# esrice/trio_binning

Measured on AMD Instinct MI355X. Metric: Gbases/sec classified (k=21, 2x300M k-mer tables), higher is better.
Workload: dtype u64

## Files before the change

### trio_binning_amd/csrc/tbk_host.cpp

```cpp
#include <hip/hip_runtime.h>

#include <fcntl.h>
#include <sys/mman.h>
#include <sys/stat.h>
#include <unistd.h>

#include <algorithm>
#include <chrono>
#include <cmath>
#include <cerrno>
#include <cstdarg>
#include <cstdio>
#include <cstdlib>
#include <cstring>
#include <cctype>
#include <pthread.h>
#include <sched.h>
#include <atomic>
#include <memory>
#include <mutex>
#include <string>
#include <thread>
#include <vector>

// ... 189 lines not shown
    buf[got] = 0;
    int n = 0;
    const char *p = buf;
    while (*p) {
        while (*p == ',' || *p == ' ' || *p == '\n') p++;
        if (!isdigit((unsigned char)*p)) break;
        char *end = nullptr;
        long lo = strtol(p, &end, 10), hi = lo;
        p = end;
        if (*p == '-') { hi = strtol(p + 1, &end, 10); p = end; }
        for (long c = lo; c <= hi && c < CPU_SETSIZE; c++) { if (cpus && n < cap) cpus[n] = (int)c; n++; }
    }
    return n;
}

extern "C" int tbk_numa_bind_thread_(int node) {
    const char *off = getenv("TBK_NUMA");
    if (off && *off == '0') return 0;
    std::vector<int> cpus(CPU_SETSIZE);
    const int n = tbk_numa_node_cpus_(node, cpus.data(), (int)cpus.size());
    if (n <= 0) return 0;
    cpu_set_t cur, want;
    if (pthread_getaffinity_np(pthread_self(), sizeof cur, &cur) != 0) return 0;
    CPU_ZERO(&want);
    for (int i = 0; i < std::min(n, (int)cpus.size()); i++) if (CPU_ISSET(cpus[(size_t)i], &cur)) CPU_SET(cpus[(size_t)i], &want);
    const int k = CPU_COUNT(&want);
    if (k == 0 || k == CPU_COUNT(&cur)) return k == 0 ? 0 : k;
    if (pthread_setaffinity_np(pthread_self(), sizeof want, &want) != 0) return 0;
    return k;
}

extern "C" int tbk_device_numa_node(int device, int *node) {
    if (!node) return fail(TBK_ERR_INVALID, "node is NULL");
    *node = -1;
    char bdf[64] = {0};
    int n_visible = 0;
    if (hipGetDeviceCount(&n_visible) != hipSuccess || n_visible <= 0) { (void)hipGetLastError(); return fail(TBK_ERR_NO_DEVICE, "no HIP device visible"); }
    if (device < 0 || device >= n_visible) return fail(TBK_ERR_INVALID, "device %d out of range (0..%d)", device, n_visible - 1);
    if (hipDeviceGetPCIBusId(bdf, (int)sizeof bdf, device) != hipSuccess) { (void)hipGetLastError(); return TBK_OK; }
    *node = tbk_numa_node_of_pci_(bdf);
    return TBK_OK;
}

extern "C" int tbk_numa_bind_to_device(int device, int *node_out, int *cpus_out) {
    int node = -1;
    const int rc = tbk_device_numa_node(device, &node);
    if (node_out) *node_out = node;
    if (cpus_out) *cpus_out = 0;
    if (rc) return rc;
    const int k = tbk_numa_bind_thread_(node);
    if (cpus_out) *cpus_out = k;
    return TBK_OK;
}

static void table_born();
static void table_gone();
struct tbk_table {
    tbk_table() { table_born(); }
    ~tbk_table() { table_gone(); }
    tbk_table(const tbk_table &) = delete;
    tbk_table &operator=(const tbk_table &) = delete;
    int device = 0;
    int k = 0;
    uint64_t num_lines = 0;
    int origin = 0;
    uint64_t *d_keys = nullptr;
    uint64_t *d_slots = nullptr;
    uint32_t n_buckets = 0;
    uint64_t distinct = 0;
    bool hashed = false;
    TbkTableView view() const { return TbkTableView{d_slots, n_buckets, 8, 0, TbkMz{0, 0, 0, 0}, 0}; }
};

struct ListRef {
    const uint64_t *d_keys;
    uint64_t num_lines;
    ListRef(const tbk_table *t) : d_keys(t->d_keys), num_lines(t->num_lines) {}
    ListRef(const uint64_t *keys, uint64_t n) : d_keys(keys), num_lines(n) {}
    const ListRef *operator->() const { return this; }
};

static constexpr int RING = 3;
static constexpr int TIMING_POOL = 4096;

struct Slot {
    uint8_t *d_bases = nullptr; size_t cap_bases = 0;
    uint64_t *d_offsets = nullptr; size_t cap_reads = 0;
    int32_t *d_counts = nullptr;
    uint8_t *h_bases = nullptr; size_t hcap_bases = 0;
    uint64_t *h_offsets = nullptr; int32_t *h_counts = nullptr; size_t hcap_reads = 0;
    uint32_t *d_codes = nullptr; uint16_t *d_bad = nullptr; size_t cap_chunks = 0;
    bool bad_clean = false;
    uint32_t *d_exc_chunk = nullptr; uint16_t *d_exc_mask = nullptr; size_t cap_exc = 0;
    uint32_t *h_codes = nullptr; size_t hcap_chunks = 0;
    uint32_t *h_exc_chunk = nullptr; uint16_t *h_exc_mask = nullptr; size_t hcap_exc = 0;
    hipEvent_t copied = nullptr, probed = nullptr, done = nullptr, copied2 = nullptr;
    hipEvent_t sliced[8] = {nullptr, nullptr, nullptr, nullptr, nullptr, nullptr, nullptr, nullptr};
    bool busy = false;
    uint64_t ticket = 0, n_reads = 0;
    int32_t *user_counts = nullptr;
    bool counts_staged = false;
};

struct DeviceStreams {
    int device = 0;
    hipStream_t compute = nullptr, copy = nullptr, out = nullptr;
    hipStream_t copy2 = nullptr;
    std::mutex enqueue;
    std::atomic<int> in_flight{0};
    ~DeviceStreams() {
        if (hipSetDevice(device) != hipSuccess) return;
        if (compute) (void)hipStreamDestroy(compute);
        if (copy) (void)hipStreamDestroy(copy);
        if (copy2) (void)hipStreamDestroy(copy2);
        if (out) (void)hipStreamDestroy(out);
    }
};

struct tbk_classifier {
    int device = 0;
    int k = 0;
    tbk_options opt = resolve_options(nullptr);
    std::shared_ptr<DeviceStreams> streams;
    uint64_t *d_pair = nullptr;
    std::shared_ptr<uint64_t> pair_owner;
    void *pair_base = nullptr;
    void own_pair() {
        const int dev = device;
        void *base = pair_base ? pair_base : (void *)d_pair;
        pair_owner = std::shared_ptr<uint64_t>(d_pair, [dev, base](uint64_t *) { if (base && hipSetDevice(dev) == hipSuccess) (void)hipFree(base); });
        pair_base = nullptr;
    }
    hipError_t alloc_pair(size_t bytes) {
        const size_t align = (size_t)opt.table_align;
        pair_base = nullptr; d_pair = nullptr;
        hipError_t e = hipMalloc(&pair_base, bytes + align);
        if (e != hipSuccess) { pair_base = nullptr; return e; }
        uintptr_t p = (uintptr_t)pair_base;
        if (align > 1) p = (p + align - 1) / align * align;
        d_pair = (uint64_t *)p;
        return hipSuccess;
    }
    void free_pair() {
        if (pair_base) (void)hipFree(pair_base);
        else if (d_pair) (void)hipFree(d_pair);
        pair_base = nullptr; d_pair = nullptr;
    }
    uint32_t n_buckets = 0;
    uint64_t distinct_a = 0, distinct_b = 0;
    uint64_t shared = 0;
    TbkMz mz{0, 0, 0};
    int replica_copies = 0;
    int layout_builds = 0;
    uint64_t past_half = 0;
    uint64_t behind_front = 0;
    uint64_t entries_a = 0, entries_b = 0;
    uint32_t guests = 0;
    uint64_t verified_lines = 0;
    double verify_s = 0;
    uint32_t over_mask = 0;
    uint64_t table_bytes() const { return (uint64_t)n_buckets * 2 * TBK_BUCKET_BYTES + ((guests & TBK_FLAG_SHORT) ? ((uint64_t)over_mask + 1) * 8 : 0); }
    TbkPairView pair() const { return TbkPairView{d_pair, n_buckets, mz, guests, over_mask}; }
    hipStream_t compute = nullptr, copy = nullptr, out = nullptr;
    Slot ring[RING];
    uint64_t next_ticket = 1;
    int max_blocks = 0;
// ... 1462 lines not shown
    if (e == hipSuccess) e = hipEventRecord(e0, c->compute);
    if (e == hipSuccess) e = tbk_launch_gather_pairs(c->d_pair, bytes, inflight, waves_per_simd, n_lines, 9, sink, &done, c->compute);
    if (e == hipSuccess) e = hipEventRecord(e1, c->compute);
    if (e == hipSuccess) e = hipEventSynchronize(e1);
    if (e == hipSuccess) e = hipEventElapsedTime(&ms, e0, e1);
    if (e0) (void)hipEventDestroy(e0);
    if (e1) (void)hipEventDestroy(e1);
    (void)hipFree(sink);
    if (e != hipSuccess) return fail(e == hipErrorInvalidValue ? TBK_ERR_INVALID : TBK_ERR_HIP, "tbk_classifier_calibrate_pairs: %s", hipGetErrorString(e));
    *lines_per_sec = ms > 0 ? (double)done / (ms * 1e-3) : 0;
    return TBK_OK;
}

extern "C" int tbk_classifier_table_id(const tbk_classifier *c, uint64_t *table_id, int *is_replica) {
    if (!c) return fail(TBK_ERR_INVALID, "classifier is NULL");
    if (table_id) *table_id = (uint64_t)(uintptr_t)c->d_pair;
    if (is_replica) *is_replica = c->replica_copies;
    return TBK_OK;
}

extern "C" int tbk_classifier_shared_keys(const tbk_classifier *c, uint64_t *n_shared) {
    if (!c || !n_shared) return fail(TBK_ERR_INVALID, "NULL argument");
    *n_shared = c->shared;
    return TBK_OK;
}

extern "C" void tbk_classifier_destroy(tbk_classifier *c) {
    if (!c) return;
    if (hipSetDevice(c->device) == hipSuccess) {
        if (c->compute) (void)hipStreamSynchronize(c->compute);
        if (c->copy) (void)hipStreamSynchronize(c->copy);
        if (c->out) (void)hipStreamSynchronize(c->out);
        for (Slot &s : c->ring) {
            if (s.d_bases) (void)hipFree(s.d_bases);
            if (s.d_offsets) (void)hipFree(s.d_offsets);
            if (s.d_counts) (void)hipFree(s.d_counts);
            if (s.h_bases) (void)hipHostFree(s.h_bases);
            if (s.h_offsets) (void)hipHostFree(s.h_offsets);
            if (s.h_counts) (void)hipHostFree(s.h_counts);
            if (s.d_codes) (void)hipFree(s.d_codes);
            if (s.d_bad) (void)hipFree(s.d_bad);
            if (s.d_exc_chunk) (void)hipFree(s.d_exc_chunk);
            if (s.d_exc_mask) (void)hipFree(s.d_exc_mask);
            if (s.h_codes) (void)hipHostFree(s.h_codes);
            if (s.h_exc_chunk) (void)hipHostFree(s.h_exc_chunk);
            if (s.h_exc_mask) (void)hipHostFree(s.h_exc_mask);
            if (s.copied) (void)hipEventDestroy(s.copied);
            if (s.probed) (void)hipEventDestroy(s.probed);
            if (s.done) (void)hipEventDestroy(s.done);
            if (s.copied2) (void)hipEventDestroy(s.copied2);
            for (hipEvent_t e : s.sliced) if (e) (void)hipEventDestroy(e);
        }
        for (hipEvent_t e : c->ev) (void)hipEventDestroy(e);
        c->pair_owner.reset();
        if (c->d_pass_read) (void)hipFree(c->d_pass_read);
        c->small_free();
        for (const Slot &s : c->ring) if (s.busy && c->streams) c->streams->in_flight--;
        c->streams.reset();
    }
    delete c;
}

static void par_memcpy(void *dst, const void *src, size_t n) {
    const size_t piece = (size_t)16 << 20;
    const int nt = (int)std::min<size_t>((size_t)tbk_host_threads(), n / piece);
    if (nt <= 1) { memcpy(dst, src, n); return; }
    std::vector<std::thread> pool;
    for (int t = 0; t < nt; t++) {
        const size_t lo = n * (size_t)t / nt, hi = n * (size_t)(t + 1) / nt;
        pool.emplace_back([=]() { memcpy((char *)dst + lo, (const char *)src + lo, hi - lo); });
    }
    for (std::thread &th : pool) th.join();
}

static bool is_pinned(const void *p) {
    hipPointerAttribute_t at;
    hipError_t e = hipPointerGetAttributes(&at, p);
    if (e != hipSuccess) { (void)hipGetLastError(); return false; }
    return at.type == hipMemoryTypeHost;
}

struct ProbeSlice { uint64_t pass_lo, pass_hi; hipEvent_t arrived; };

static int launch_probe_timed(tbk_classifier *c, const uint8_t *d_bases, const uint64_t *d_offsets,
                              uint64_t n_reads, uint64_t total, int32_t *d_counts, const uint32_t *d_codes = nullptr,
                              const uint16_t *d_bad16 = nullptr, const ProbeSlice *slices = nullptr, int n_slices = 0) {
    if (n_reads >= 0xFFFFFFF0ull) return fail(TBK_ERR_INVALID, "more than 2^32 reads in one batch");
    if (total == 0) {
        HIP_TRY(hipMemsetAsync(d_counts, 0, n_reads * 2 * sizeof(int32_t), c->compute));
        return TBK_OK;
    }
    const uint64_t passes = tbk_probe_passes(total);
    if (passes > c->cap_passes) {
        HIP_TRY(hipStreamSynchronize(c->compute));
        if (c->d_pass_read) HIP_TRY(hipFree(c->d_pass_read));
        c->d_pass_read = nullptr; c->cap_passes = 0;
        const uint64_t cap = (passes + passes / 4 + 1024 + 1) & ~1ull;
        HIP_TRY(hipMalloc((void **)&c->d_pass_read, (4 * cap + 16) * sizeof(uint32_t)));
        c->cap_passes = cap;
    }
    const ProbeSlice whole = {0, passes, nullptr};
    if (n_slices <= 0) { slices = &whole; n_slices = 1; }
    hipEvent_t *ev = nullptr;
    if (c->timing) {
        const size_t need = 2 + 3 * (size_t)n_slices;
        if (c->ev_used + need > c->ev.size() && c->ev.size() >= (size_t)TIMING_POOL) {
            HIP_TRY(hipStreamSynchronize(c->compute));
            int rc = c->fold_timing();
            if (rc) return rc;
        }
        while (c->ev_used + need > c->ev.size()) {
            hipEvent_t a;
            HIP_TRY(hipEventCreate(&a));
            c->ev.push_back(a);
        }
        ev = c->ev.data() + c->ev_used;
        c->ev_used += need;
        c->ev_slices.push_back((uint32_t)n_slices);
        c->timed_launches++;
        HIP_TRY(hipEventRecord(ev[0], c->compute));
    }
    HIP_TRY(tbk_launch_probe_index(d_offsets, n_reads, total, d_counts, c->d_pass_read, c->cap_passes, c->opt.two_read_kernel != 0 && tbk_probe_has_two_read_kernel(c->mz), c->compute));
    if (ev) HIP_TRY(hipEventRecord(ev[1], c->compute));
    for (int j = 0; j < n_slices; j++) {
        if (slices[j].arrived) HIP_TRY(hipStreamWaitEvent(c->compute, slices[j].arrived, 0));
        if (ev) HIP_TRY(hipEventRecord(ev[2 + 3 * j], c->compute));
        HIP_TRY(tbk_launch_probe_range(d_bases, d_codes, d_bad16, d_offsets, n_reads, total, c->pair(), c->k, d_counts, c->d_pass_read, c->cap_passes,
                                       slices[j].pass_lo, slices[j].pass_hi, c->max_blocks, c->opt.two_read_kernel != 0, ev ? ev[3 + 3 * j] : nullptr, c->compute, 0));
        if (ev) HIP_TRY(hipEventRecord(ev[4 + 3 * j], c->compute));
    }
    c->last_passes = passes;
    return TBK_OK;
}

int tbk_classifier::fold_timing() {
    size_t at = 0;
    for (uint32_t n_slices : ev_slices) {
        float ms = 0;
        HIP_TRY(hipEventElapsedTime(&ms, ev[at], ev[at + 1]));
        timed_ms += ms;
        for (uint32_t j = 0; j < n_slices; j++) {
            float whole = 0, single = 0;
            HIP_TRY(hipEventElapsedTime(&whole, ev[at + 2 + 3 * j], ev[at + 4 + 3 * j]));
            HIP_TRY(hipEventElapsedTime(&single, ev[at + 3 + 3 * j], ev[at + 4 + 3 * j]));
            timed_ms += whole;
            timed_single_ms += single;
        }
        at += 2 + 3 * (size_t)n_slices;
    }
    ev_used = 0;
    ev_slices.clear();
    return TBK_OK;
}

extern "C" int tbk_stream_depth(const tbk_classifier *) { return RING; }

extern "C" int tbk_check_offsets_(const uint64_t *offsets, uint64_t n_reads) {
    if (!offsets) return fail(TBK_ERR_INVALID, "offsets is NULL");
    if (offsets[0] != 0) return fail(TBK_ERR_INVALID, "offsets[0] must be 0");
    for (uint64_t i = 0; i < n_reads; i++)
        if (offsets[i + 1] < offsets[i]) return fail(TBK_ERR_INVALID, "offsets not non-decreasing at read %llu", (unsigned long long)i);
    return TBK_OK;
}

static int slot_reserve_device(Slot &s, uint64_t total, uint64_t n_reads) {
    const size_t need_b = ((size_t)total + 15) & ~(size_t)15;
    if (need_b > s.cap_bases) {
        if (s.d_bases) HIP_TRY(hipFree(s.d_bases));
        s.d_bases = nullptr; s.cap_bases = 0;
        const size_t cap = std::max(need_b + need_b / 8, (size_t)1 << 20);
        HIP_TRY(hipMalloc((void **)&s.d_bases, cap));
        s.cap_bases = cap;
    }
    if (n_reads > s.cap_reads) {
        if (s.d_offsets) HIP_TRY(hipFree(s.d_offsets));
        if (s.d_counts) HIP_TRY(hipFree(s.d_counts));
        s.d_offsets = nullptr; s.d_counts = nullptr; s.cap_reads = 0;
        const size_t cap = std::max((size_t)n_reads + (size_t)n_reads / 8, (size_t)1024);
        HIP_TRY(hipMalloc((void **)&s.d_offsets, (cap + 1) * sizeof(uint64_t)));
        HIP_TRY(hipMalloc((void **)&s.d_counts, cap * 2 * sizeof(int32_t)));
        s.cap_reads = cap;
    }
    return TBK_OK;
}

static int slot_reserve(Slot &s, uint64_t stage_bases, uint64_t n_reads, bool stage_small, bool stage_out) {
    const size_t need_b = ((size_t)stage_bases + 15) & ~(size_t)15;
    if (need_b > s.hcap_bases) {
        if (s.h_bases) HIP_TRY(hipHostFree(s.h_bases));
        s.h_bases = nullptr; s.hcap_bases = 0;
        const size_t cap = std::max(need_b + need_b / 8, (size_t)1 << 20);
        HIP_TRY(hipHostMalloc((void **)&s.h_bases, cap, hipHostMallocPortable));
        s.hcap_bases = cap;
    }
    if ((stage_small || stage_out) && n_reads > s.hcap_reads) {
        if (s.h_offsets) HIP_TRY(hipHostFree(s.h_offsets));
        if (s.h_counts) HIP_TRY(hipHostFree(s.h_counts));
        s.h_offsets = nullptr; s.h_counts = nullptr; s.hcap_reads = 0;
        const size_t cap = std::max((size_t)n_reads + (size_t)n_reads / 8, (size_t)1024);
        HIP_TRY(hipHostMalloc((void **)&s.h_offsets, (cap + 1) * sizeof(uint64_t), hipHostMallocPortable));
        HIP_TRY(hipHostMalloc((void **)&s.h_counts, cap * 2 * sizeof(int32_t), hipHostMallocPortable));
        s.hcap_reads = cap;
    }
    return TBK_OK;
}

static int slot_reserve_packed(Slot &s, uint64_t n_chunks, uint64_t n_exc) {
    if (n_chunks > s.cap_chunks) {
        if (s.d_codes) HIP_TRY(hipFree(s.d_codes));
        if (s.d_bad) HIP_TRY(hipFree(s.d_bad));
        s.d_codes = nullptr; s.d_bad = nullptr; s.cap_chunks = 0;
        const size_t cap = std::max((size_t)n_chunks + (size_t)n_chunks / 8, (size_t)1 << 16);
        HIP_TRY(hipMalloc((void **)&s.d_codes, cap * sizeof(uint32_t)));
        HIP_TRY(hipMalloc((void **)&s.d_bad, (cap + 2) * sizeof(uint16_t)));
        s.cap_chunks = cap;
        s.bad_clean = false;
    }
    if (n_exc > s.cap_exc) {
        if (s.d_exc_chunk) HIP_TRY(hipFree(s.d_exc_chunk));
        if (s.d_exc_mask) HIP_TRY(hipFree(s.d_exc_mask));
        s.d_exc_chunk = nullptr; s.d_exc_mask = nullptr; s.cap_exc = 0;
        const size_t cap = std::max((size_t)n_exc + (size_t)n_exc / 4, (size_t)4096);
        HIP_TRY(hipMalloc((void **)&s.d_exc_chunk, cap * sizeof(uint32_t)));
        HIP_TRY(hipMalloc((void **)&s.d_exc_mask, cap * sizeof(uint16_t)));
        s.cap_exc = cap;
    }
    return TBK_OK;
}

static int slot_reserve_packed_host(Slot &s, uint64_t n_chunks, uint64_t n_exc) {
    if (n_chunks > s.hcap_chunks) {
// ... 8 lines not shown
        if (s.h_exc_mask) HIP_TRY(hipHostFree(s.h_exc_mask));
        s.h_exc_chunk = nullptr; s.h_exc_mask = nullptr; s.hcap_exc = 0;
        const size_t cap = std::max((size_t)n_exc + (size_t)n_exc / 4, (size_t)4096);
        HIP_TRY(hipHostMalloc((void **)&s.h_exc_chunk, cap * sizeof(uint32_t), hipHostMallocPortable));
        HIP_TRY(hipHostMalloc((void **)&s.h_exc_mask, cap * sizeof(uint16_t), hipHostMallocPortable));
        s.hcap_exc = cap;
    }
    return TBK_OK;
}

static int submit_host(tbk_classifier *c, const uint8_t *bases, const uint32_t *codes, const uint32_t *exc_chunk, const uint16_t *exc_mask,
                       uint64_t n_exc, const uint64_t *offsets, uint64_t n_reads, int32_t *counts, uint64_t *ticket) {
    if (!c || !offsets || !ticket || (n_reads && !counts)) return fail(TBK_ERR_INVALID, "NULL argument");
    int rc = tbk_check_offsets_(offsets, n_reads);
    if (rc) return rc;
    const uint64_t total = offsets[n_reads];
    if (total && !bases && !codes) return fail(TBK_ERR_INVALID, "bases is NULL");
    if (codes && n_exc && (!exc_chunk || !exc_mask)) return fail(TBK_ERR_INVALID, "exception arrays are NULL");
    rc = use_device(c->device);
    if (rc) return rc;
    const uint64_t tk = c->next_ticket;
    Slot &s = c->ring[tk % RING];
    if (s.busy) return fail(TBK_ERR_STATE, "all %d stream slots are in flight; call tbk_stream_wait(%llu) first", RING,
                            (unsigned long long)s.ticket);
    const uint64_t n_chunks = tbk_packed_chunks(total);
    bool packed = codes != nullptr;
    if (!packed && total && c->packed_h2d) {
        rc = slot_reserve_packed_host(s, n_chunks, 0);
        if (rc) return rc;
        rc = tbk_pack_bases_vec(bases, total, s.h_codes, c->exc_chunk, c->exc_mask, c->pack_threads);
        if (rc) return fail(rc, "%s", g_err.c_str());
        n_exc = c->exc_chunk.size();
        rc = slot_reserve_packed_host(s, n_chunks, n_exc);
        if (rc) return rc;
        if (n_exc) {
            memcpy(s.h_exc_chunk, c->exc_chunk.data(), n_exc * sizeof(uint32_t));
            memcpy(s.h_exc_mask, c->exc_mask.data(), n_exc * sizeof(uint16_t));
        }
        codes = s.h_codes; exc_chunk = s.h_exc_chunk; exc_mask = s.h_exc_mask;
        packed = true;
    } else if (packed && total) {
        const bool codes_pinned = is_pinned(codes), exc_pinned = n_exc == 0 || (is_pinned(exc_chunk) && is_pinned(exc_mask));
        rc = slot_reserve_packed_host(s, codes_pinned ? 0 : n_chunks, exc_pinned ? 0 : n_exc);
        if (rc) return rc;
        if (!codes_pinned) { par_memcpy(s.h_codes, codes, n_chunks * sizeof(uint32_t)); codes = s.h_codes; }
        if (!exc_pinned) {
            memcpy(s.h_exc_chunk, exc_chunk, n_exc * sizeof(uint32_t));
            memcpy(s.h_exc_mask, exc_mask, n_exc * sizeof(uint16_t));
            exc_chunk = s.h_exc_chunk; exc_mask = s.h_exc_mask;
        }
        for (uint64_t i = 0; i < n_exc; i++)
            if (exc_chunk[i] >= n_chunks) return fail(TBK_ERR_INVALID, "exception %llu names chunk %u of %llu", (unsigned long long)i, exc_chunk[i], (unsigned long long)n_chunks);
    }
    const bool bases_pinned = packed || total == 0 || is_pinned(bases);
    const bool offs_pinned = is_pinned(offsets);
    const bool out_pinned = n_reads == 0 || is_pinned(counts);
    rc = slot_reserve(s, bases_pinned ? 0 : total, n_reads, !bases_pinned || !offs_pinned, !out_pinned);
    if (rc) return rc;
    rc = slot_reserve_device(s, packed ? 0 : total, n_reads);
    if (rc) return rc;
    if (packed) {
        rc = slot_reserve_packed(s, n_chunks, n_exc);
        if (rc) return rc;
    }
    s.ticket = tk; s.n_reads = n_reads; s.user_counts = counts; s.counts_staged = !out_pinned;
    if (n_reads && total) {
        const uint64_t *src_o = offsets;
        if (!offs_pinned) { memcpy(s.h_offsets, offsets, (n_reads + 1) * sizeof(uint64_t)); src_o = s.h_offsets; }
        const uint8_t *src_b = bases;
        if (!packed && !bases_pinned) { par_memcpy(s.h_bases, bases, total); src_b = s.h_bases; }
        std::lock_guard<std::mutex> together(c->streams->enqueue);
        HIP_TRY(hipMemcpyAsync(s.d_offsets, src_o, (n_reads + 1) * sizeof(uint64_t), hipMemcpyHostToDevice, c->copy));
        if (packed) {
            if (!s.bad_clean) HIP_TRY(hipMemsetAsync(s.d_bad, 0, (s.cap_chunks + 2) * sizeof(uint16_t), c->copy));
            s.bad_clean = false;
            if (n_exc) {
                HIP_TRY(hipMemcpyAsync(s.d_exc_chunk, exc_chunk, n_exc * sizeof(uint32_t), hipMemcpyHostToDevice, c->copy));
                HIP_TRY(hipMemcpyAsync(s.d_exc_mask, exc_mask, n_exc * sizeof(uint16_t), hipMemcpyHostToDevice, c->copy));
            }
        }
        HIP_TRY(hipEventRecord(s.copied, c->copy));
        const uint64_t passes = tbk_probe_passes(total);
        const bool zero_copy = packed && c->opt.zero_copy != 0 && is_pinned(codes);
        const bool alone = c->streams->in_flight.load() == 0;
        const int n_slices = alone ? (int)std::max<uint64_t>(1, std::min<uint64_t>(8, total / c->slice_bases)) : 1;
        ProbeSlice slices[8];
        uint64_t sent = 0;
        for (int j = 0; j < n_slices; j++) {
            slices[j].pass_lo = passes * (uint64_t)j / (uint64_t)n_slices;
            slices[j].pass_hi = passes * (uint64_t)(j + 1) / (uint64_t)n_slices;
            slices[j].arrived = s.sliced[j];
            const uint64_t upto = j + 1 == n_slices ? n_chunks : std::min<uint64_t>(n_chunks, slices[j].pass_hi * (TBK_PASS_BASES / 16) + 2);
            if (upto > sent) {
                if (packed && zero_copy) {
                } else if (packed && n_slices == 1 && c->streams->copy2 && upto - sent >= ((uint64_t)1 << 22)) {
                    const uint64_t mid = sent + (upto - sent) / 2;
                    HIP_TRY(hipMemcpyAsync(s.d_codes + mid, codes + mid, (upto - mid) * sizeof(uint32_t), hipMemcpyHostToDevice, c->streams->copy2));
                    HIP_TRY(hipEventRecord(s.copied2, c->streams->copy2));
                    HIP_TRY(hipMemcpyAsync(s.d_codes + sent, codes + sent, (mid - sent) * sizeof(uint32_t), hipMemcpyHostToDevice, c->copy));
                    HIP_TRY(hipStreamWaitEvent(c->copy, s.copied2, 0));
                } else if (packed) {
                    HIP_TRY(hipMemcpyAsync(s.d_codes + sent, codes + sent, (upto - sent) * sizeof(uint32_t), hipMemcpyHostToDevice, c->copy));
                } else {
                    const uint64_t b0 = sent * 16, b1 = std::min<uint64_t>(total, upto * 16);
                    HIP_TRY(hipMemcpyAsync(s.d_bases + b0, src_b + b0, b1 - b0, hipMemcpyHostToDevice, c->copy));
                }
                sent = upto;
            }
            HIP_TRY(hipEventRecord(s.sliced[j], c->copy));
        }
        HIP_TRY(hipStreamWaitEvent(c->compute, s.copied, 0));
        if (packed) HIP_TRY(tbk_launch_scatter_bad(s.d_exc_chunk, s.d_exc_mask, n_exc, s.d_bad, total, 0, c->compute));
        rc = launch_probe_timed(c, packed ? nullptr : s.d_bases, s.d_offsets, n_reads, total, s.d_counts, packed ? (zero_copy ? const_cast<uint32_t *>(codes) : s.d_codes) : nullptr,
                                packed ? s.d_bad : nullptr, slices, n_slices);
        if (rc) return rc;
        if (packed) {
            HIP_TRY(tbk_launch_scatter_bad(s.d_exc_chunk, s.d_exc_mask, n_exc, s.d_bad, total, 1, c->compute));
            s.bad_clean = true;
        }
        HIP_TRY(hipEventRecord(s.probed, c->compute));
        HIP_TRY(hipStreamWaitEvent(c->out, s.probed, 0));
        HIP_TRY(hipMemcpyAsync(out_pinned ? counts : s.h_counts, s.d_counts, n_reads * 2 * sizeof(int32_t),
                               hipMemcpyDeviceToHost, c->out));
        HIP_TRY(hipEventRecord(s.done, c->out));
    } else {
        if (n_reads) memset(counts, 0, n_reads * 2 * sizeof(int32_t));
        s.counts_staged = false;
        HIP_TRY(hipEventRecord(s.done, c->compute));
    }
    s.busy = true;
    c->streams->in_flight++;
    c->next_ticket++;
    *ticket = tk;
    return TBK_OK;
}

extern "C" int tbk_stream_submit(tbk_classifier *c, const uint8_t *bases, const uint64_t *offsets, uint64_t n_reads,
                                 int32_t *counts, uint64_t *ticket) {
    return submit_host(c, bases, nullptr, nullptr, nullptr, 0, offsets, n_reads, counts, ticket);
}

extern "C" int tbk_stream_submit_packed(tbk_classifier *c, const uint32_t *codes, const uint32_t *exc_chunk, const uint16_t *exc_mask,
                                        uint64_t n_exc, const uint64_t *offsets, uint64_t n_reads, int32_t *counts, uint64_t *ticket) {
    if (!codes && offsets && n_reads && offsets[n_reads]) return fail(TBK_ERR_INVALID, "codes is NULL");
    static const uint32_t none = 0;
    return submit_host(c, nullptr, codes ? codes : &none, exc_chunk, exc_mask, n_exc, offsets, n_reads, counts, ticket);
}

extern "C" int tbk_classifier_set_transfer(tbk_classifier *c, int packed) {
    if (!c) return fail(TBK_ERR_INVALID, "classifier is NULL");
    c->packed_h2d = packed != 0;
    return TBK_OK;
}

extern "C" int tbk_classifier_transfer(const tbk_classifier *c) { return c ? c->packed_h2d : -1; }

extern "C" int tbk_classifier_set_pack_threads_(tbk_classifier *c, int threads) {
    if (!c) return fail(TBK_ERR_INVALID, "classifier is NULL");
    c->pack_threads = threads > 0 ? threads : 0;
    return TBK_OK;
}

extern "C" int tbk_stream_wait(tbk_classifier *c, uint64_t ticket) {
    if (!c) return fail(TBK_ERR_INVALID, "classifier is NULL");
    Slot &s = c->ring[ticket % RING];
    if (!s.busy || s.ticket != ticket) return fail(TBK_ERR_STATE, "ticket %llu is not in flight", (unsigned long long)ticket);
    int rc = use_device(c->device);
    if (rc) return rc;
    HIP_TRY(hipEventSynchronize(s.done));
// ... 811 lines not shown
```

### trio_binning_amd/csrc/tbk_kernels.hip

```cpp
#include <hip/hip_runtime.h>
#include <stdint.h>

#include <algorithm>
#include <type_traits>

#include "tbk_common.h"
#include "tbk_device.h"

__device__ __forceinline__ bool tbk_lookup_slow(const TbkTableView t, uint64_t key) {
    if (key >= TBK_NOKEY) return false;
    uint32_t b = tbk_bucket_of(key, t.mz, t.n_buckets);
    for (uint32_t walked = 0; walked <= t.n_buckets; walked++) {
        const uint64_t *line = t.slots + (uint64_t)b * t.stride;
        for (uint32_t s = 0; s < TBK_SLOTS_PER_BUCKET; s++)
            if (line[tbk_slot_at(t.guests, t.stride, t.half, s)] == key) return true;
        if (t.stride == 16 && (t.guests & (TBK_FLAG_FRONT | TBK_FLAG_GUESTS)) == (TBK_FLAG_FRONT | TBK_FLAG_GUESTS))
            for (uint32_t s = 0; s < 4; s++)
                if (line[tbk_slot_at(t.guests, t.stride, t.half ^ 8u, s)] == (key | TBK_GUEST)) return true;
        if (!(line[tbk_slot_at(t.guests, t.stride, t.half, 6)] > line[tbk_slot_at(t.guests, t.stride, t.half, 7)])) return false;
        if (t.guests & TBK_FLAG_GUESTS) {
            for (uint32_t s = 0; s < TBK_SLOTS_PER_BUCKET; s++)
                if (line[tbk_slot_at(t.guests, t.stride, t.half ^ 8u, s)] == (key | TBK_GUEST)) return true;
            if (!(line[tbk_slot_at(t.guests, t.stride, t.half, 4)] > line[tbk_slot_at(t.guests, t.stride, t.half, 5)])) return false;
        }
// ... 1826 lines not shown
}

extern "C" hipError_t tbk_launch_insert(uint64_t *slots, uint32_t n_buckets, uint32_t stride, uint32_t half, TbkMz mz,
                                        const uint64_t *d_keys, uint64_t n, uint32_t *d_overflowed, uint32_t *d_left_line, uint32_t guests, TbkTableView skip,
                                        unsigned long long *d_distinct, unsigned long long *d_skipped, int *d_failed,
                                        hipStream_t stream) {
    if (n == 0) return hipSuccess;
    uint64_t blocks = (n + 255) / 256;
    if (blocks > 65536) blocks = 65536;
    hipLaunchKernelGGL(tbk_insert_kernel, dim3((unsigned)blocks), dim3(256), 0, stream, slots, n_buckets, stride,
                       half, mz, d_keys, n, d_overflowed, d_left_line, guests, skip, d_distinct, d_skipped, d_skipped + 1, d_failed);
    return hipGetLastError();
}

extern "C" hipError_t tbk_launch_order(uint64_t *slots, uint64_t n_halves, const uint32_t *d_overflowed, const uint32_t *d_left_line,
                                       uint32_t flags, uint32_t stride, hipStream_t stream) {
    if (n_halves == 0) return hipSuccess;
    hipLaunchKernelGGL(tbk_order_kernel, dim3((unsigned)((n_halves + 255) / 256)), dim3(256), 0, stream, slots, n_halves, d_overflowed, d_left_line, flags, stride);
    return hipGetLastError();
}

extern "C" hipError_t tbk_launch_contains(TbkTableView t, const uint64_t *d_keys, uint64_t n,
                                          uint8_t *d_out, hipStream_t stream) {
    if (n == 0) return hipSuccess;
    hipLaunchKernelGGL(tbk_contains_kernel, dim3((unsigned)((n + 255) / 256)), dim3(256), 0, stream, t,
                       d_keys, n, d_out);
    return hipGetLastError();
}

__global__ void __launch_bounds__(256)
tbk_scatter_bad_kernel(const uint32_t *__restrict__ exc_chunk, const uint16_t *__restrict__ exc_mask, uint64_t n,
                       uint16_t *__restrict__ bad16, uint64_t total, int clear) {
    const uint64_t i = (uint64_t)blockIdx.x * blockDim.x + threadIdx.x;
    uint32_t *words = reinterpret_cast<uint32_t *>(bad16);
    if (i < n) {
        const uint32_t c = exc_chunk[i];
        if (clear) atomicAnd(&words[c >> 1], ~(0xFFFFu << (16 * (c & 1u))));
        else atomicOr(&words[c >> 1], (uint32_t)exc_mask[i] << (16 * (c & 1u)));
    }
    if (i == 0 && (total & 15u) != 0) {
        const uint64_t c = total >> 4;
        if (clear) atomicAnd(&words[c >> 1], ~(0xFFFFu << (16 * (c & 1u))));
        else atomicOr(&words[c >> 1], ((0xFFFFu << (total & 15u)) & 0xFFFFu) << (16 * (c & 1u)));
    }
}

extern "C" hipError_t tbk_launch_scatter_bad(const uint32_t *d_exc_chunk, const uint16_t *d_exc_mask, uint64_t n, uint16_t *d_bad16,
                                             uint64_t total, int clear, hipStream_t stream) {
    if (n == 0 && (total & 15u) == 0) return hipSuccess;
    hipLaunchKernelGGL(tbk_scatter_bad_kernel, dim3((unsigned)((std::max<uint64_t>(n, 1) + 255) / 256)), dim3(256), 0, stream, d_exc_chunk, d_exc_mask, n, d_bad16, total, clear);
    return hipGetLastError();
}

static void fill_args(ProbeArgs &p, const uint8_t *d_bases, const uint32_t *d_codes, const uint16_t *d_bad16, const uint64_t *d_offsets,
                      uint64_t n_reads, uint64_t total, TbkPairView t, int k, int32_t *d_counts, uint32_t *d_scratch, uint64_t pass_cap) {
    p.codes = d_codes; p.bad16 = d_bad16; p.n_chunks = (total + 15) / 16;
    p.bases = d_bases; p.offsets = d_offsets; p.n_reads = n_reads; p.total = total;
    p.n_passes = (total + TBK_PASS - 1) / TBK_PASS;
    p.t = t; p.k = k; p.counts = d_counts; p.pass_read = d_scratch; p.multi_list = d_scratch + pass_cap; p.two_list = (const uint64_t *)(d_scratch + 2 * pass_cap);
    p.n_multi = d_scratch + 4 * pass_cap; p.n_two = d_scratch + 4 * pass_cap + 1;
    p.pass_lo = 0; p.pass_hi = p.n_passes;
}

extern "C" int tbk_probe_has_two_read_kernel(TbkMz mz) { return mz.w >= 2 && mz.t > 0; }

extern "C" hipError_t tbk_launch_probe_index(const uint64_t *d_offsets, uint64_t n_reads, uint64_t total, int32_t *d_counts, uint32_t *d_scratch,
                                             uint64_t pass_cap, int use_two, hipStream_t stream) {
    if (total == 0 || n_reads == 0) return hipSuccess;
    const uint64_t n_passes = (total + TBK_PASS - 1) / TBK_PASS;
    if (n_passes > pass_cap) return hipErrorInvalidValue;
    uint32_t *d_multi = d_scratch + pass_cap, *d_n = d_scratch + 4 * pass_cap;
    uint64_t *d_two = (uint64_t *)(d_scratch + 2 * pass_cap);
    if (pass_cap & 1) return hipErrorInvalidValue;
    hipError_t e = hipMemsetAsync(d_n, 0, 2 * sizeof(uint32_t), stream);
    if (e != hipSuccess) return e;
    hipLaunchKernelGGL(tbk_pass_index_kernel, dim3((unsigned)((n_passes + 1023) / 1024)), dim3(1024), 0, stream,
                       d_offsets, n_reads, total, n_passes, d_scratch, d_multi, d_n, d_two, d_n + 1, use_two, d_counts);
    return hipGetLastError();
}

extern "C" hipError_t tbk_launch_probe_range(const uint8_t *d_bases, const uint32_t *d_codes, const uint16_t *d_bad16, const uint64_t *d_offsets,
                                             uint64_t n_reads, uint64_t total, TbkPairView t, int k, int32_t *d_counts, uint32_t *d_scratch,
                                             uint64_t pass_cap, uint64_t pass_lo, uint64_t pass_hi, int max_blocks, int use_two, hipEvent_t between, hipStream_t stream,
                                             int only_single) {
    if (total == 0 || n_reads == 0 || pass_hi <= pass_lo) return hipSuccess;
    ProbeArgs p;
    fill_args(p, d_bases, d_codes, d_bad16, d_offsets, n_reads, total, t, k, d_counts, d_scratch, pass_cap);
    if (p.n_passes > pass_cap || pass_hi > p.n_passes) return hipErrorInvalidValue;
    p.pass_lo = pass_lo; p.pass_hi = pass_hi;
    const uint64_t blocks = (pass_hi - pass_lo + TBK_WAVES_PER_BLOCK - 1) / TBK_WAVES_PER_BLOCK;
    uint64_t blocks_multi = std::min<uint64_t>(blocks, 16384);
    if (max_blocks > 0 && blocks_multi > (uint64_t)max_blocks) blocks_multi = (uint64_t)max_blocks;
    const dim3 grid((unsigned)blocks), grid_multi((unsigned)blocks_multi), block(64 * TBK_WAVES_PER_BLOCK);
    const bool m64 = t.mz.m > 16, samp = t.mz.t > 0, front = (t.guests & TBK_FLAG_FRONT) != 0, entry = (t.guests & TBK_FLAG_ENTRY) != 0;
    if (front && t.mz.w < 2) return hipErrorInvalidValue;
    const bool wide = (t.guests & TBK_FLAG_WIDE) != 0, shortk = (t.guests & TBK_FLAG_SHORT) != 0, fullk = (t.guests & TBK_FLAG_FULL) != 0;
    const bool span3 = (entry || shortk) && t.mz.t > 0 && t.mz.t == t.mz.m - 2 * t.mz.w;
    if ((entry || shortk) && t.mz.t > 0 && !span3 && t.mz.t != t.mz.m - t.mz.w) return hipErrorInvalidValue;
    if (TBK_TMER_LUT && span3 && t.mz.w == 6 && t.mz.t != 4) return hipErrorInvalidValue;
    if (shortk) {
        TbkShortGeom g;
        if (!tbk_short_geom(k, t.mz, t.n_buckets, &g) || t.n_buckets > 0x3FFFFFFFu) return hipErrorInvalidValue;
    }
    if (fullk && (!tbk_full_geom(k, t.mz) || t.mz.t != t.mz.m - t.mz.w || t.n_buckets > 0x3FFFFFFFu)) return hipErrorInvalidValue;
    if (entry) {
        TbkEntryGeom g;
        if (!(wide ? tbk_wentry_geom(k, t.mz, &g) : tbk_entry_geom(k, t.mz, &g)) || t.n_buckets > 0x3FFFFFFFu) return hipErrorInvalidValue;
    }
    const uint64_t blocks_two = use_two && tbk_probe_has_two_read_kernel(t.mz) ? std::min<uint64_t>(n_reads > 1 ? n_reads - 1 : 0, p.n_passes) : 0;
    const dim3 grid_two((unsigned)std::max<uint64_t>(1, blocks_two));
    hipError_t e = hipSuccess;
    for (int which = 2; which >= 0; which--) {
        if (which == 1 && blocks_two == 0) continue;
        if (which != 0 && only_single) continue;
        if (which == 0 && between != nullptr) { e = hipEventRecord(between, stream); if (e != hipSuccess) return e; }
#define TBK_LAUNCH(N, M, S, F) do { if (which == 2) hipLaunchKernelGGL((tbk_probe_kernel<N, M, S, F, true>), grid_multi, block, 0, stream, p); \
                                    else if (which == 0) hipLaunchKernelGGL((tbk_probe_kernel<N, M, S, F, false>), grid, block, 0, stream, p); \
                                    else if (S && N >= 2) hipLaunchKernelGGL((tbk_probe_kernel<N, M, (S && N >= 2), F, false, (S && N >= 2)>), grid_two, block, 0, stream, p); } while (0)
#define TBK_W(N) case N: if (samp && front) { if (m64) TBK_LAUNCH(N, true, true, true); else TBK_LAUNCH(N, false, true, true); } \
                         else if (samp) { if (m64) TBK_LAUNCH(N, true, true, false); else TBK_LAUNCH(N, false, true, false); } \
                         else if (front) { if (m64) TBK_LAUNCH(N, true, false, true); else TBK_LAUNCH(N, false, false, true); } \
                         else { if (m64) TBK_LAUNCH(N, true, false, false); else TBK_LAUNCH(N, false, false, false); } break;
        if (entry || shortk || fullk) {
#define TBK_E1(N, WD, LW) do { if (which == 2) hipLaunchKernelGGL((tbk_probe_entry_kernel<N, true, false, WD, LW>), grid_multi, block, 0, stream, p); \
                         else if (which == 0) hipLaunchKernelGGL((tbk_probe_entry_kernel<N, false, false, WD, LW>), grid, block, 0, stream, p); \
                         else hipLaunchKernelGGL((tbk_probe_entry_kernel<N, false, true, WD, LW>), grid_two, block, 0, stream, p); } while (0)
#define TBK_E(N, WD) case N: if (span3) TBK_E1(N, WD, 3); else TBK_E1(N, WD, 2); break;
#define TBK_E2(N, WD) case N: if (span3) return hipErrorInvalidValue; TBK_E1(N, WD, 2); break;
            if (fullk) {
                switch (t.mz.w) {
#ifdef TBK_ONLY_W6
                    TBK_E2(6, 3) TBK_E2(8, 3)
#else
                    TBK_E2(2, 3) TBK_E2(3, 3) TBK_E2(4, 3) TBK_E2(5, 3) TBK_E2(6, 3) TBK_E2(7, 3) TBK_E2(8, 3)
#endif
                    default: return hipErrorInvalidValue;
                }
            } else if (shortk) {
                switch (t.mz.w) {
#ifdef TBK_ONLY_W6
                    TBK_E(6, 2)
#else
                    TBK_E(2, 2) TBK_E(3, 2) TBK_E(4, 2) TBK_E(5, 2) TBK_E(6, 2) TBK_E2(7, 2) TBK_E2(8, 2)
#endif
                    default: return hipErrorInvalidValue;
                }
            } else if (wide) {
                switch (t.mz.w) {
#ifdef TBK_ONLY_W6
                    TBK_E2(6, 1) TBK_E2(8, 1)
#else
                    TBK_E2(2, 1) TBK_E2(3, 1) TBK_E2(4, 1) TBK_E2(5, 1) TBK_E2(6, 1) TBK_E2(7, 1) TBK_E2(8, 1)
#endif
                    default: return hipErrorInvalidValue;
                }
            } else {
                switch (t.mz.w) {
#ifdef TBK_ONLY_W6
                    TBK_E(6, 0)
#else
                    TBK_E(2, 0) TBK_E(3, 0) TBK_E(4, 0) TBK_E(5, 0) TBK_E(6, 0) TBK_E2(7, 0)
#endif
                    default: return hipErrorInvalidValue;
                }
            }
#undef TBK_E
#undef TBK_E2
#undef TBK_E1
            e = hipGetLastError();
            if (e != hipSuccess) return e;
            continue;
        }
        switch (t.mz.w) {
#ifdef TBK_ONLY_W6
            TBK_W(6)
#else
            case 0: TBK_LAUNCH(0, false, false, false); break;
            case 1: if (m64) TBK_LAUNCH(1, true, false, false); else TBK_LAUNCH(1, false, false, false); break;
            TBK_W(2) TBK_W(3) TBK_W(4) TBK_W(5) TBK_W(6) TBK_W(7) TBK_W(8)
#endif
            default: return hipErrorInvalidValue;
        }
#undef TBK_W
#undef TBK_LAUNCH
        e = hipGetLastError();
        if (e != hipSuccess) return e;
    }
    return hipSuccess;
}

#ifdef TBK_COUNTERS
extern "C" int tbk_debug_counters(unsigned long long out[8], int reset) {
    hipError_t e = hipMemcpyFromSymbol(out, HIP_SYMBOL(tbk_dbg), 8 * sizeof(unsigned long long));
    if (e == hipSuccess && reset) {
        unsigned long long z[8] = {0, 0, 0, 0, 0, 0, 0, 0};
        e = hipMemcpyToSymbol(HIP_SYMBOL(tbk_dbg), z, sizeof z);
    }
// ... 6 lines not shown
```

Measured before the change: 220.3.

## Slice single-read probe per copy arrival and defer multi-pass kernels to one tail launch

When a batch is split into slices, each slice now runs only the single-read probe kernel as its bases arrive. The multi-read and two-read kernels run once over the whole pass range after all slices, instead of once per slice. Slicing is also enabled even when other batches are in flight, and the slice count is capped by a compile-time constant (default 4 instead of 8). The aim is to overlap more of the copy with compute and to cut repeated launches of the multi-pass kernels, at the cost of the multi kernels waiting until the whole batch has arrived.

```diff
diff --git a/trio_binning_amd/csrc/tbk_host.cpp b/trio_binning_amd/csrc/tbk_host.cpp
--- a/trio_binning_amd/csrc/tbk_host.cpp
+++ b/trio_binning_amd/csrc/tbk_host.cpp
@@ -295,6 +295,11 @@
 
 static constexpr int RING = 3;
 static constexpr int TIMING_POOL = 4096;
+#ifndef TBK_SLICE_CAP
+#define TBK_SLICE_CAP 4
+#endif
+static constexpr int SLICE_CAP = TBK_SLICE_CAP;
+static_assert(SLICE_CAP >= 1 && SLICE_CAP <= 8, "Slot::sliced holds 8 events");
 
 struct Slot {
     uint8_t *d_bases = nullptr; size_t cap_bases = 0;
@@ -1923,6 +1928,8 @@
 
 struct ProbeSlice { uint64_t pass_lo, pass_hi; hipEvent_t arrived; };
 
+static size_t timing_events(int n_slices) { return n_slices == 1 ? 5 : 4 + 2 * (size_t)n_slices; }
+
 static int launch_probe_timed(tbk_classifier *c, const uint8_t *d_bases, const uint64_t *d_offsets,
                               uint64_t n_reads, uint64_t total, int32_t *d_counts, const uint32_t *d_codes = nullptr,
                               const uint16_t *d_bad16 = nullptr, const ProbeSlice *slices = nullptr, int n_slices = 0) {
@@ -1944,7 +1951,7 @@
     if (n_slices <= 0) { slices = &whole; n_slices = 1; }
     hipEvent_t *ev = nullptr;
     if (c->timing) {
-        const size_t need = 2 + 3 * (size_t)n_slices;
+        const size_t need = timing_events(n_slices);
         if (c->ev_used + need > c->ev.size() && c->ev.size() >= (size_t)TIMING_POOL) {
             HIP_TRY(hipStreamSynchronize(c->compute));
             int rc = c->fold_timing();
@@ -1961,14 +1968,27 @@
         c->timed_launches++;
         HIP_TRY(hipEventRecord(ev[0], c->compute));
     }
-    HIP_TRY(tbk_launch_probe_index(d_offsets, n_reads, total, d_counts, c->d_pass_read, c->cap_passes, c->opt.two_read_kernel != 0 && tbk_probe_has_two_read_kernel(c->mz), c->compute));
+    const int use_two = c->opt.two_read_kernel != 0;
+    HIP_TRY(tbk_launch_probe_index(d_offsets, n_reads, total, d_counts, c->d_pass_read, c->cap_passes, use_two && tbk_probe_has_two_read_kernel(c->mz), c->compute));
     if (ev) HIP_TRY(hipEventRecord(ev[1], c->compute));
-    for (int j = 0; j < n_slices; j++) {
-        if (slices[j].arrived) HIP_TRY(hipStreamWaitEvent(c->compute, slices[j].arrived, 0));
-        if (ev) HIP_TRY(hipEventRecord(ev[2 + 3 * j], c->compute));
+    if (n_slices == 1) {
+        if (slices[0].arrived) HIP_TRY(hipStreamWaitEvent(c->compute, slices[0].arrived, 0));
+        if (ev) HIP_TRY(hipEventRecord(ev[2], c->compute));
         HIP_TRY(tbk_launch_probe_range(d_bases, d_codes, d_bad16, d_offsets, n_reads, total, c->pair(), c->k, d_counts, c->d_pass_read, c->cap_passes,
-                                       slices[j].pass_lo, slices[j].pass_hi, c->max_blocks, c->opt.two_read_kernel != 0, ev ? ev[3 + 3 * j] : nullptr, c->compute, 0));
-        if (ev) HIP_TRY(hipEventRecord(ev[4 + 3 * j], c->compute));
+                                       slices[0].pass_lo, slices[0].pass_hi, c->max_blocks, use_two, ev ? ev[3] : nullptr, c->compute, 0));
+        if (ev) HIP_TRY(hipEventRecord(ev[4], c->compute));
+    } else {
+        for (int j = 0; j < n_slices; j++) {
+            if (slices[j].arrived) HIP_TRY(hipStreamWaitEvent(c->compute, slices[j].arrived, 0));
+            if (ev) HIP_TRY(hipEventRecord(ev[2 + 2 * j], c->compute));
+            HIP_TRY(tbk_launch_probe_range(d_bases, d_codes, d_bad16, d_offsets, n_reads, total, c->pair(), c->k, d_counts, c->d_pass_read, c->cap_passes,
+                                           slices[j].pass_lo, slices[j].pass_hi, c->max_blocks, use_two, nullptr, c->compute, 1));
+            if (ev) HIP_TRY(hipEventRecord(ev[3 + 2 * j], c->compute));
+        }
+        if (ev) HIP_TRY(hipEventRecord(ev[2 + 2 * n_slices], c->compute));
+        HIP_TRY(tbk_launch_probe_range(d_bases, d_codes, d_bad16, d_offsets, n_reads, total, c->pair(), c->k, d_counts, c->d_pass_read, c->cap_passes,
+                                       0, passes, c->max_blocks, use_two, nullptr, c->compute, 2));
+        if (ev) HIP_TRY(hipEventRecord(ev[3 + 2 * n_slices], c->compute));
     }
     c->last_passes = passes;
     return TBK_OK;
@@ -1980,14 +2000,21 @@
         float ms = 0;
         HIP_TRY(hipEventElapsedTime(&ms, ev[at], ev[at + 1]));
         timed_ms += ms;
-        for (uint32_t j = 0; j < n_slices; j++) {
+        if (n_slices == 1) {
             float whole = 0, single = 0;
-            HIP_TRY(hipEventElapsedTime(&whole, ev[at + 2 + 3 * j], ev[at + 4 + 3 * j]));
-            HIP_TRY(hipEventElapsedTime(&single, ev[at + 3 + 3 * j], ev[at + 4 + 3 * j]));
+            HIP_TRY(hipEventElapsedTime(&whole, ev[at + 2], ev[at + 4]));
+            HIP_TRY(hipEventElapsedTime(&single, ev[at + 3], ev[at + 4]));
             timed_ms += whole;
             timed_single_ms += single;
+        } else {
+            for (uint32_t j = 0; j <= n_slices; j++) {
+                float part = 0;
+                HIP_TRY(hipEventElapsedTime(&part, ev[at + 2 + 2 * j], ev[at + 3 + 2 * j]));
+                timed_ms += part;
+                if (j < n_slices) timed_single_ms += part;
+            }
         }
-        at += 2 + 3 * (size_t)n_slices;
+        at += timing_events((int)n_slices);
     }
     ev_used = 0;
     ev_slices.clear();
@@ -2162,9 +2189,8 @@
         HIP_TRY(hipEventRecord(s.copied, c->copy));
         const uint64_t passes = tbk_probe_passes(total);
         const bool zero_copy = packed && c->opt.zero_copy != 0 && is_pinned(codes);
-        const bool alone = c->streams->in_flight.load() == 0;
-        const int n_slices = alone ? (int)std::max<uint64_t>(1, std::min<uint64_t>(8, total / c->slice_bases)) : 1;
-        ProbeSlice slices[8];
+        const int n_slices = (int)std::max<uint64_t>(1, std::min<uint64_t>(SLICE_CAP, total / c->slice_bases));
+        ProbeSlice slices[SLICE_CAP];
         uint64_t sent = 0;
         for (int j = 0; j < n_slices; j++) {
             slices[j].pass_lo = passes * (uint64_t)j / (uint64_t)n_slices;
diff --git a/trio_binning_amd/csrc/tbk_kernels.hip b/trio_binning_amd/csrc/tbk_kernels.hip
--- a/trio_binning_amd/csrc/tbk_kernels.hip
+++ b/trio_binning_amd/csrc/tbk_kernels.hip
@@ -1932,7 +1932,7 @@
 extern "C" hipError_t tbk_launch_probe_range(const uint8_t *d_bases, const uint32_t *d_codes, const uint16_t *d_bad16, const uint64_t *d_offsets,
                                              uint64_t n_reads, uint64_t total, TbkPairView t, int k, int32_t *d_counts, uint32_t *d_scratch,
                                              uint64_t pass_cap, uint64_t pass_lo, uint64_t pass_hi, int max_blocks, int use_two, hipEvent_t between, hipStream_t stream,
-                                             int only_single) {
+                                             int part) {
     if (total == 0 || n_reads == 0 || pass_hi <= pass_lo) return hipSuccess;
     ProbeArgs p;
     fill_args(p, d_bases, d_codes, d_bad16, d_offsets, n_reads, total, t, k, d_counts, d_scratch, pass_cap);
@@ -1962,7 +1962,8 @@
     hipError_t e = hipSuccess;
     for (int which = 2; which >= 0; which--) {
         if (which == 1 && blocks_two == 0) continue;
-        if (which != 0 && only_single) continue;
+        if (which != 0 && part == 1) continue;
+        if (which == 0 && part == 2) continue;
         if (which == 0 && between != nullptr) { e = hipEventRecord(between, stream); if (e != hipSuccess) return e; }
 #define TBK_LAUNCH(N, M, S, F) do { if (which == 2) hipLaunchKernelGGL((tbk_probe_kernel<N, M, S, F, true>), grid_multi, block, 0, stream, p); \
                                     else if (which == 0) hipLaunchKernelGGL((tbk_probe_kernel<N, M, S, F, false>), grid, block, 0, stream, p); \
```

Result: no change. 219.6 (-0.3%).
